# POSTECH-CVLab/PyTorch-StudioGAN

Measured on AMD Instinct MI355X. Metric: images/sec (G+D step) BigGAN ImageNet-128 bs256, higher is better.
Workload: dtype bf16

## Files before the change

include/sgamd.h:

```cpp
#ifndef SGAMD_H
#define SGAMD_H
#include <stdint.h>
#ifdef __cplusplus
extern "C" {
#endif

typedef void* sg_stream_t;

#define SG_DTYPE_F32 0
#define SG_DTYPE_BF16 1
#define SG_DTYPE_F64 2

#define SG_PIX_RELU 1
#define SG_PIX_UPSAMPLE 2
#define SG_PIX_QUAD 4
#define SG_PIX_TRANSPOSED 8
#define SG_EPI_OUT_F32 1
#define SG_EPI_ATOMIC 2
#define SG_EPI_POOL 4
#define SG_EPI_RELU 8
#define SG_EPI_RES_F32 16

const char* sg_last_error(void);
int sg_version(void);
// ... 185 lines not shown
  const float* w;
  const float* u; const float* v; const float* sigma;
  float* dw;
  int rows, cols, Cin, RS, natural, apply_sn, trans;
  int Cin_pad;
} sg_sn_bwd_layer;
int sg_sn_backward(const sg_sn_bwd_layer* layers_dev, const sg_sn_bwd_layer* layers_host, int n, float* work, long long work_floats, sg_stream_t s);

int sg_embedding_fwd(const float* table, const int64_t* idx, float* out, int B, int dim, int num, sg_stream_t s);
int sg_embedding_bwd(const float* dout, const int64_t* idx, float* dtable, int B, int dim, int num, sg_stream_t s);
int sg_relu_sum_hw_fwd(int dtype, const void* x, float* h, int B, int HW, int C, sg_stream_t s);
int sg_relu_sum_hw_bwd(int dtype, const void* x, const float* dh, void* dx, int B, int HW, int C, sg_stream_t s);
int sg_pd_head_fwd(const float* h, const float* w1, const float* b1, const float* emb, float* adv, int B, int C, sg_stream_t s);
int sg_pd_head_bwd(const float* h, const float* w1, const float* emb, const float* dadv, float* dh, float* dw1, float* db1,
                   float* demb, int B, int C, sg_stream_t s);
int sg_loss_d(int kind, const float* real, const float* fake, int B, float* loss, float* d_real, float* d_fake, sg_stream_t s);
int sg_loss_g(int kind, const float* fake, int B, float* loss, float* d_fake, sg_stream_t s);

int sg_interp_rows(const float* real, const float* fake, const float* alpha, float* out, int B, long long n, sg_stream_t s);
int sg_gp_fwd(int kind, const float* grads, int B, long long n, float* norms, float* loss, sg_stream_t s);
int sg_gp_bwd(int kind, const float* grads, const float* norms, const float* gout, float* dgrads, int B, long long n, sg_stream_t s);
int sg_masked_sum_hw(int dtype, const void* t, const void* x, float* out, int B, int HW, int C, sg_stream_t s);

int sg_attn_fused_ok(int B, int HW, int HW4, int Dp, int Cg);
int sg_attn_fwd_fused_ok(int B, int HW, int HW4, int Dp, int Cg);
int sg_attn_fwd_flash_ok(int B, int HW, int HW4, int Dp, int Cg);
int sg_attn_fwd_fused(const void* theta, const void* phi, const void* g, void* P, float* lse, void* O, float* O32, int B, int HW, int HW4, int Dp, int Cg, sg_stream_t s);
int sg_attn_bwd_fused_ok(int B, int HW, int HW4, int Dp, int Cg);
int sg_attn_bwd_fused(const void* theta, const void* phi, const void* g, const void* dO, const float* O32, const float* lse, float* delta, void* dtheta, void* dphi,
                      void* dg, int B, int HW, int HW4, int Dp, int Cg, sg_stream_t s);
int sg_attn_probs_fwd(const void* theta, const void* phi, void* P, float* lse, int B, int HW, int HW4, int Dp, sg_stream_t s);
int sg_attn_ds_bwd(const void* theta, const void* phi, const void* g, const void* dO, const float* lse, void* dS,
                   int B, int HW, int HW4, int Dp, int Cg, sg_stream_t s);

int sg_slice_up_fwd(int dtype, const void* x, void* y, int N, int Hs, int Ws, int ldx, int C, int up, sg_stream_t s);
int sg_slice_up_bwd(int dtype, const void* dy, void* dx, int N, int Hs, int Ws, int ldx, int C, int up, sg_stream_t s);
int sg_copy_channels(int dtype, const void* src, int ld_src, void* dst, int ld_dst, long long rows, int C, sg_stream_t s);

int sg_adam_ema(float* p, const float* g, float* m, float* v, float* ema, long long n, float lr, float beta1, float beta2,
                float eps, float wd, int step, float ema_decay, float grad_scale, sg_stream_t s);
int sg_ema_lerp(const float* src, float* ema, long long n, float decay, sg_stream_t s);

int sg_lecam(const float* real, const float* fake, int B, float ema_real, float ema_fake, float* loss, float* d_real, float* d_fake, sg_stream_t s);
int sg_u8_to_nhwc(int dtype, const uint8_t* x, const uint8_t* flip, void* y, int N, int H, int W, int cpad, sg_stream_t s);

int sg_quantize_resize_normalize(int dtype, const float* x, void* out, uint8_t* quant_out, int N, int C, int H, int W,
                                 int OH, int OW, int quantize, sg_stream_t s);
int sg_pool2d(int dtype, const void* x, void* y, int N, int H, int W, int C, int k, int stride, int pad, int mode, int ldy, int c_off, sg_stream_t s);
int sg_pil_resize_normalize(int dtype, const float* x, void* out, float* tmp, int N, int C, int H, int W, int OH, int OW,
                            const int* bounds_h, const double* kk_h, int ksize_h, const int* bounds_v, const double* kk_v, int ksize_v,
                            int quantize, sg_stream_t s);
int sg_global_avgpool(int dtype, const void* x, float* y, int N, int HW, int C, sg_stream_t s);
int sg_topk_hits(const float* scores, int ld, int ncls, const int64_t* labels, int k, int N, uint8_t* hits, sg_stream_t s);
int sg_topk_select(const float* x, int n, int k, float* vals, int* idx, sg_stream_t s);
int sg_topk_scatter(const float* g, const int* idx, int k, float* dx, int n, sg_stream_t s);
int sg_feat_moments_accumulate(const float* f, int n, int C, double* sum_f, double* sum_ff, sg_stream_t s);
int sg_gather_images_u8(const uint8_t* src, const int64_t* idx, const uint8_t* flip, uint8_t* dst, int B, int H, int W,
                        const int64_t* lab_src, int64_t* lab_dst, sg_stream_t s);
int sg_row_normalize_fwd(const float* x, float* y, float* inv, int rows, int cols, float eps, sg_stream_t s);
int sg_row_normalize_bwd(const float* y, const float* inv, const float* dy, float* dx, int rows, int cols, sg_stream_t s);
int sg_row_dot(const float* a, const float* b, float* p, int rows, int cols, sg_stream_t s);
int sg_row_scale(const float* g, const float* x, float* out, int rows, int cols, int accumulate, sg_stream_t s);
int sg_class_loss(int kind, const float* z, const int64_t* label, int rows, int cols, float* row_loss, float* loss, float* dz, sg_stream_t s);
int sg_contrastive_loss(int kind, const float* S, const float* p, const int64_t* label, int B, float temperature, float m_p,
                        float* row_loss, float* loss, float* dS, float* dp, sg_stream_t s);
int sg_gather_cols(const float* z, const int64_t* label, int rows, int cols, float* out, sg_stream_t s);
// ... 67 lines not shown
```

pytorch-studiogan_amd/_lib.py:

```python
import ctypes as C
import os
import subprocess
import sys

import torch

_HERE = os.path.dirname(os.path.abspath(__file__))
LIB_PATH = os.path.join(_HERE, "libsgamd.so")
if os.environ.get("SG_LIBSGAMD"):
    LIB_PATH = os.path.abspath(os.environ["SG_LIBSGAMD"])
CSRC = os.path.join(_HERE, "csrc")

F32, BF16, F64 = 0, 1, 2
PIX_RELU, PIX_UPSAMPLE, PIX_QUAD, PIX_TRANSPOSED = 1, 2, 4, 8
Q_POOL, Q_UP = 0, 1
EPI_OUT_F32, EPI_ATOMIC, EPI_POOL, EPI_RELU, EPI_RES_F32 = 1, 2, 4, 8, 16

_vp, _i, _f, _ll = C.c_void_p, C.c_int, C.c_float, C.c_longlong


class ConvFwdDesc(C.Structure):
    _fields_ = [("dtype", _i), ("N", _i), ("Hs", _i), ("Ws", _i), ("C", _i), ("ldx", _i), ("Ho", _i), ("Wo", _i), ("Cout", _i),
                ("R", _i), ("S", _i), ("stride", _i), ("pad_h", _i), ("pad_w", _i), ("pix_flags", _i), ("epi_flags", _i),
                ("alpha", _f), ("beta", _f), ("x", _vp), ("w", _vp), ("bias", _vp), ("res", _vp), ("mask", _vp), ("out", _vp),
# ... 116 lines not shown
    "sg_comm_size": [_vp, C.POINTER(_i)],
    "sg_comm_destroy": [_vp],
    "sg_allreduce_flat": [_vp, _vp, _ll, _i, _vp],
    "sg_bn_stats_sync": [_i, _vp, _i, _ll, _i, _vp, _vp, _f, _f, _vp, _vp, _vp, _vp, _vp],
    "sg_set_f32_mode": [_i],
    "sg_get_f32_mode": [],
    "sg_reduce_scatter_flat": [_vp, _vp, _ll, _vp],
    "sg_allgather_flat": [_vp, _vp, _ll, _vp],
    "sg_p2p_create": [_i, _i, _ll, C.POINTER(_vp), _vp],
    "sg_p2p_connect": [_vp, _vp],
    "sg_p2p_destroy": [_vp],
    "sg_p2p_timeouts": [_vp, C.POINTER(_i)],
    "sg_p2p_allreduce_f64": [_vp, _vp, _i, _vp],
    "sg_bn_finalize_p2p": [_vp, _vp, C.c_double, _i, _f, _f, _vp, _vp, _vp, _vp, _vp],
    "sg_bn_stats_sync_p2p": [_i, _vp, _i, _ll, _i, _vp, _vp, _f, _f, _vp, _vp, _vp, _vp, _vp],
    "sg_bn_from_running": [_vp, _vp, _i, _f, _vp, _vp, _vp],
    "sg_bn_apply": [_i, _vp, _vp, _i, _ll, _i, _vp, _vp, _vp, _vp, _i, _i, _vp],
    "sg_bn_bwd_reduce": [_i, _vp, _vp, _i, _ll, _i, _vp, _vp, _vp, _vp, _i, _i, _vp, _vp],
    "sg_bn_bwd_finalize": [_vp, _i, _i, _vp, _i, _vp, _vp, _vp, _vp],
    "sg_bn_bwd_apply": [_i, _vp, _vp, _vp, _i, _ll, _i, _vp, _vp, _vp, _vp, _i, _i, _vp, C.c_double, _i, _vp],
    "sg_bn_bwd_apply_res": [_i, _vp, _vp, _vp, _i, _ll, _i, _vp, _vp, _vp, _vp, _i, _i, _vp, C.c_double, _i, _vp, _vp],
    "sg_bn_bwd2_reduce": [_i, _vp, _vp, _vp, _i, _ll, _i, _vp, _vp, _vp, _vp, _i, _vp, _vp],
    "sg_bn_bwd2_finalize": [_vp, _i, _i, _vp, _vp],
    "sg_bn_bwd2_dgain": [_vp, _vp, C.c_double, _vp, _i, _i, _vp, _vp],
    "sg_bn_bwd2_apply": [_i, _vp, _vp, _vp, _vp, _vp, _i, _ll, _i, _vp, _vp, _vp, _vp, _i, _vp, C.c_double, _i, _vp],
    "sg_attn_fused_ok": [_i, _i, _i, _i, _i],
    "sg_attn_fwd_fused_ok": [_i, _i, _i, _i, _i],
    "sg_attn_fwd_flash_ok": [_i, _i, _i, _i, _i],
    "sg_attn_fwd_fused": [_vp, _vp, _vp, _vp, _vp, _vp, _vp, _i, _i, _i, _i, _i, _vp],
    "sg_attn_bwd_fused_ok": [_i, _i, _i, _i, _i],
    "sg_attn_bwd_fused": [_vp, _vp, _vp, _vp, _vp, _vp, _vp, _vp, _vp, _vp, _i, _i, _i, _i, _i, _vp],
    "sg_attn_probs_fwd": [_vp, _vp, _vp, _vp, _i, _i, _i, _i, _vp],
    "sg_attn_ds_bwd": [_vp, _vp, _vp, _vp, _vp, _vp, _i, _i, _i, _i, _i, _vp],
    "sg_slice_up_fwd": [_i, _vp, _vp, _i, _i, _i, _i, _i, _i, _vp],
    "sg_slice_up_bwd": [_i, _vp, _vp, _i, _i, _i, _i, _i, _i, _vp],
    "sg_copy_channels": [_i, _vp, _i, _vp, _i, _ll, _i, _vp],
    "sg_interp_rows": [_vp, _vp, _vp, _vp, _i, _ll, _vp],
    "sg_gp_fwd": [_i, _vp, _i, _ll, _vp, _vp, _vp],
    "sg_gp_bwd": [_i, _vp, _vp, _vp, _vp, _i, _ll, _vp],
    "sg_masked_sum_hw": [_i, _vp, _vp, _vp, _i, _i, _i, _vp],
    "sg_sn_forward": [_i, _vp, C.POINTER(SnLayer), _i, _f, _vp, _ll, _vp],
    "sg_sn_backward": [_vp, C.POINTER(SnBwdLayer), _i, _vp, _ll, _vp],
    "sg_embedding_fwd": [_vp, _vp, _vp, _i, _i, _i, _vp],
    "sg_embedding_bwd": [_vp, _vp, _vp, _i, _i, _i, _vp],
    "sg_relu_sum_hw_fwd": [_i, _vp, _vp, _i, _i, _i, _vp],
    "sg_relu_sum_hw_bwd": [_i, _vp, _vp, _vp, _i, _i, _i, _vp],
    "sg_pd_head_fwd": [_vp, _vp, _vp, _vp, _vp, _i, _i, _vp],
    "sg_pd_head_bwd": [_vp, _vp, _vp, _vp, _vp, _vp, _vp, _vp, _i, _i, _vp],
    "sg_loss_d": [_i, _vp, _vp, _i, _vp, _vp, _vp, _vp],
    "sg_loss_g": [_i, _vp, _i, _vp, _vp, _vp],
    "sg_adam_ema": [_vp, _vp, _vp, _vp, _vp, _ll, _f, _f, _f, _f, _f, _i, _f, _f, _vp],
    "sg_ema_lerp": [_vp, _vp, _ll, _f, _vp],
    "sg_quantize_resize_normalize": [_i, _vp, _vp, _vp, _i, _i, _i, _i, _i, _i, _i, _vp],
    "sg_pil_resize_normalize": [_i, _vp, _vp, _vp, _i, _i, _i, _i, _i, _i, _vp, _vp, _i, _vp, _vp, _i, _i, _vp],
    "sg_pool2d": [_i, _vp, _vp, _i, _i, _i, _i, _i, _i, _i, _i, _i, _i, _vp],
    "sg_global_avgpool": [_i, _vp, _vp, _i, _i, _i, _vp],
    "sg_feat_moments_accumulate": [_vp, _i, _i, _vp, _vp, _vp],
    "sg_topk_hits": [_vp, _i, _i, _vp, _i, _i, _vp, _vp],
    "sg_row_normalize_fwd": [_vp, _vp, _vp, _i, _i, _f, _vp],
    "sg_row_normalize_bwd": [_vp, _vp, _vp, _vp, _i, _i, _vp],
    "sg_row_dot": [_vp, _vp, _vp, _i, _i, _vp],
    "sg_row_scale": [_vp, _vp, _vp, _i, _i, _i, _vp],
    "sg_class_loss": [_i, _vp, _vp, _i, _i, _vp, _vp, _vp, _vp],
    "sg_contrastive_loss": [_i, _vp, _vp, _vp, _i, _f, _f, _vp, _vp, _vp, _vp, _vp],
    "sg_gather_cols": [_vp, _vp, _i, _i, _vp, _vp],
    "sg_scatter_cols": [_vp, _vp, _i, _i, _vp, _vp],
# ... 120 lines not shown
```

pytorch-studiogan_amd/functional/attention.py:

```python
from ._base import *
from .layout import ConvertFn
from .conv import ConvCfg, ConvDgradFn

class MaxPool2Fn(torch.autograd.Function):

    @staticmethod
    def forward(ctx, x):
        x = _c(x)
        B, H, W, Cc = x.shape
        y = torch.empty((B, (H // 2) * (W // 2), Cc), dtype=x.dtype, device=x.device)
        idx = torch.empty((B, (H // 2) * (W // 2), Cc), dtype=torch.uint8, device=x.device)
        L.call("sg_maxpool2_fwd", L.dt(x), L.ptr(x), Cc, L.ptr(y), Cc, L.ptr(idx), B, H, W, Cc, L.stream())
        ctx.save_for_backward(idx)
        ctx.dims = (B, H, W, Cc)
        return y

    @staticmethod
    def backward(ctx, dy):
        (idx,) = ctx.saved_tensors
        if torch.is_grad_enabled():
            return MaxPool2BwdFn.apply(dy, idx, ctx.dims)
        return _maxpool2_bwd(dy, idx, ctx.dims)


def _maxpool2_bwd(dy, idx, dims):
    B, H, W, Cc = dims
    dy = _c(dy)
    dx = torch.empty((B, H, W, Cc), dtype=dy.dtype, device=dy.device)
    L.call("sg_maxpool2_bwd", L.dt(dy), L.ptr(dy), Cc, L.ptr(idx), L.ptr(dx), Cc, B, H, W, Cc, L.stream())
    return dx


class MaxPool2BwdFn(torch.autograd.Function):
    @staticmethod
    def forward(ctx, dy, idx, dims):
# ... 177 lines not shown
                ins = [t for t, need in zip((theta, phi, g), ctx.needs_input_grad) if need]
                grads = list(torch.autograd.grad(_attn_reference_graph(theta, phi, g, ctx.dims), ins, do, create_graph=True)) if ins else []
            return tuple(grads.pop(0) if need else None for need in ctx.needs_input_grad)
        HW, HW4 = H * W, (H // 2) * (W // 2)
        do = _c(do)
        dev, T = do.device, do.dtype
        sd = L.dt(T)
        if P is None:
            assert lse is not None
            delta = torch.empty((B, HW), dtype=torch.float32, device=dev)
            dtheta = torch.empty((B, H, W, Dp), dtype=T, device=dev)
            dphi = torch.empty((B, HW4, Dp), dtype=T, device=dev)
            dg = torch.empty((B, HW4, Cg), dtype=T, device=dev)
            L.call("sg_attn_bwd_fused", L.ptr(theta), L.ptr(phi), L.ptr(g), L.ptr(do), L.ptr(o32), L.ptr(lse), L.ptr(delta), L.ptr(dtheta), L.ptr(dphi),
                   L.ptr(dg), B, HW, HW4, Dp, Cg, L.stream())
            return dtheta, dphi, dg
        dg = torch.empty((B, HW4, Cg), dtype=T, device=dev)
        gemm_raw(sd, do, 1, Cg, P, 1, HW4, dg, Cg, Cg, HW4, HW, batch=B, p_bs=HW * Cg, q_bs=HW * HW4, out_bs=HW4 * Cg)
        dS = torch.empty((B, HW, HW4), dtype=T, device=dev)
        if lse is not None:
            L.call("sg_attn_ds_bwd", L.ptr(theta), L.ptr(phi), L.ptr(g), L.ptr(do), L.ptr(lse), L.ptr(dS), B, HW, HW4, Dp, Cg, L.stream())
        else:
            dP = torch.empty((B, HW, HW4), dtype=torch.float32, device=dev)
            gemm_raw(sd, g, 0, Cg, do, 0, Cg, dP, HW4, HW4, HW, Cg, batch=B, p_bs=HW4 * Cg, q_bs=HW * Cg, out_bs=HW * HW4, epi_flags=L.EPI_OUT_F32)
            L.call("sg_softmax_rows_bwd", sd, L.ptr(P), L.ptr(dP), L.ptr(dS), B * HW, HW4, L.stream())
            del dP
        dtheta = torch.empty((B, H, W, Dp), dtype=T, device=dev)
        gemm_raw(sd, phi, 1, Dp, dS, 0, HW4, dtheta, Dp, Dp, HW, HW4, batch=B, p_bs=HW4 * Dp, q_bs=HW * HW4, out_bs=HW * Dp)
        dphi = torch.empty((B, HW4, Dp), dtype=T, device=dev)
        gemm_raw(sd, theta, 1, Dp, dS, 1, HW4, dphi, Dp, Dp, HW4, HW, batch=B, p_bs=HW * Dp, q_bs=HW * HW4, out_bs=HW4 * Dp)
        return dtheta, dphi, dg


class AttnOutFn(torch.autograd.Function):

    @staticmethod
    def forward(ctx, x, o, weight, sigma, rt, slot, link=None):
        bank = rt.bank()
        x, o = _c(x), _c(o)
        ctx.link = link
        y = conv2d_raw(o, bank.w_fwd(slot, rt), rt.Cin, rt.rows, 1, 1, res=x, alpha_ptr=sigma)
        ctx.save_for_backward(o, sigma)
        ctx.rt, ctx.slot = rt, slot
        ctx.sigma_param = sigma
        ctx.weight = weight
        return y

    @staticmethod
    def backward(ctx, dy):
        o, sigma = ctx.saved_tensors
        rt, slot = ctx.rt, ctx.slot
        if torch.is_grad_enabled():
            if _param_grad_wanted(ctx.weight, ctx.sigma_param):
                raise NotImplementedError("create_graph=True is supported for input gradients only (WGAN-GP / R1 path)")
            do = ScalePtrFn.apply(ConvDgradFn.apply(dy, o, ctx.weight, rt, slot, ConvCfg(1, 1)), ctx.sigma_param) if ctx.needs_input_grad[1] else None
            return (dy if ctx.needs_input_grad[0] else None), do, None, None, None, None, None
        bank = rt.bank()
        dy = _c(dy)
        N, H, W, Cc = dy.shape
        do = None
        if ctx.needs_input_grad[3]:
            t = conv2d_raw(o, bank.w_fwd(slot, rt), rt.Cin, rt.rows, 1, 1)
            g = ensure_grad(ctx.sigma_param)
            L.call("sg_dot", L.dt(dy), L.ptr(dy), L.ptr(t), dy.numel(), L.ptr(g), 1.0, None, L.stream())
        if ctx.needs_input_grad[1]:
            do = conv2d_raw(dy, bank.w_dgrad(slot, rt), rt.rows, rt.Cin, 1, 1, alpha_ptr=sigma)
        if ctx.needs_input_grad[2]:
            conv2d_wgrad_raw(o, dy, bank.dwt(slot, rt), rt.Cin, rt.rows, 1, 1, H, W, alpha_ptr=sigma)
        dx = dy
        if ctx.link is not None and ctx.link.pending > 0 and ctx.needs_input_grad[0]:
            ctx.link.dx, dx = dy, None
        return dx, do, None, None, None, None, None


__all__ = ['AttnCoreFn', 'AttnOutFn', 'AttnPooledFn', 'BmmFn', 'MaxPool2BwdFn', 'MaxPool2Fn', 'ScalePtrFn', 'SoftmaxRowsBwdFn', 'SoftmaxRowsFn', '_attn_reference_graph', '_maxpool2_bwd']
```

pytorch-studiogan_amd/ops.py:

```python
import torch
import torch.nn as nn
from torch.nn import init
import torch.nn.functional as F_

from . import functional as F
from .bank import get_bank

COMPUTE_DTYPE = torch.float32


def to_nhwc(x, dtype, cpad=0):
    if x.dim() != 4:
        raise RuntimeError("expected a 4-D NCHW tensor")
    if x.dtype == torch.uint8:
        return F.u8_to_nhwc(x, dtype, max(cpad, 3))
    if cpad > x.shape[1]:
        return F.NchwToNhwcFn.apply(x.float(), dtype, cpad)
    if x.dtype == dtype and x.is_contiguous(memory_format=torch.channels_last) and not (x.shape[1] > 1 and x.is_contiguous() and x.shape[2] * x.shape[3] > 1):
        return x.permute(0, 2, 3, 1)
    if x.dtype == torch.float32 and x.is_contiguous():
        return F.NchwToNhwcFn.apply(x, dtype)
    y = x.permute(0, 2, 3, 1).contiguous()
    if y.dtype != dtype:
        y = F.ConvertFn.apply(y, dtype)
# ... 228 lines not shown
            rt_g, rt_b = self.gain._sg_rt, self.bias._sg_rt
            slot = slot if slot is not None else rt_g.bank().current
            gb = F.CbnAffineFn.apply(y, self.gain.master_weight, self.bias.master_weight, rt_g, rt_b, slot, self._ones2)
            return self.bn.forward_nhwc(x, gb, None, relu, link, packed=True)
        gain = self.gain.forward_rt(y, slot, const_bias=self._ones)
        bias = self.bias.forward_rt(y, slot)
        return self.bn.forward_nhwc(x, gain, bias, relu, link)

    def forward(self, x, y):
        _, bank = _root_and_bank(self.gain)
        if self.gain.__dict__.get("_sg_root") is None:
            raise RuntimeError("ConditionalBatchNorm2d must live inside a studiogan_amd backbone (its two linears share the network's bank)")
        return to_nchw(self.forward_nhwc(to_nhwc(x, bank.dtype), y))


class SelfAttention(nn.Module):

    def __init__(self, in_channels, is_generator, MODULES):
        super().__init__()
        self.in_channels = in_channels
        conv = MODULES.g_conv2d if is_generator else MODULES.d_conv2d
        c8, c2 = in_channels // 8, in_channels // 2
        pad8 = (c8 + 7) // 8 * 8
        self.conv1x1_theta = conv(in_channels=in_channels, out_channels=c8, kernel_size=1, stride=1, padding=0, bias=False)
        self.conv1x1_phi = conv(in_channels=in_channels, out_channels=c8, kernel_size=1, stride=1, padding=0, bias=False)
        self.conv1x1_g = conv(in_channels=in_channels, out_channels=c2, kernel_size=1, stride=1, padding=0, bias=False)
        self.conv1x1_attn = conv(in_channels=c2, out_channels=in_channels, kernel_size=1, stride=1, padding=0, bias=False)
        for m in (self.conv1x1_theta, self.conv1x1_phi):
            m._sg_rows_pad = pad8
        self.sigma = nn.Parameter(torch.zeros(1), requires_grad=True)

    def forward_nhwc(self, x, slot=None):
        link = F.GradLink(chain=True) if (F._GRAD_LINK[0] and torch.is_grad_enabled() and x.requires_grad) else None
        theta = self.conv1x1_theta.forward_nhwc(x, slot, link=link)
        phi = self.conv1x1_phi.forward_nhwc(x, slot, link=link)
        g = self.conv1x1_g.forward_nhwc(x, slot, link=link)
        o = F.AttnCoreFn.apply(theta, phi, g)
        rt = self.conv1x1_attn._sg_rt
        slot = slot if slot is not None else rt.bank().current
        return F.AttnOutFn.apply(x, o, self.conv1x1_attn.master_weight, self.sigma, rt, slot, link)

    def forward(self, x):
        _, bank = _root_and_bank(self.conv1x1_theta)
        return to_nchw(self.forward_nhwc(to_nhwc(x, bank.dtype)))


class LeCamEMA(object):

    def __init__(self, init=7777, decay=0.9, start_iter=0):
        self.G_loss = init
        self.D_loss_real = init
        self.D_loss_fake = init
        self.D_real = init
        self.D_fake = init
        self.decay = decay
        self.start_itr = start_iter

    def update(self, cur, mode, itr):
        decay = 0.0 if itr < self.start_itr else self.decay
        if mode not in ("G_loss", "D_loss_real", "D_loss_fake", "D_real", "D_fake"):
            raise ValueError(mode)
        setattr(self, mode, getattr(self, mode) * decay + cur * (1 - decay))


def conv2d(in_channels, out_channels, kernel_size, stride=1, padding=0, dilation=1, groups=1, bias=True):
    return Conv2d(in_channels, out_channels, kernel_size, stride, padding, dilation, groups, bias, sn=False)


def snconv2d(in_channels, out_channels, kernel_size, stride=1, padding=0, dilation=1, groups=1, bias=True):
    return Conv2d(in_channels, out_channels, kernel_size, stride, padding, dilation, groups, bias, sn=True)


# ... 83 lines not shown
```

Measured before the change: 2031.

## Fuse attention theta/phi/g 1x1 projections with 2x2 max-pool into one kernel

Adds an MFMA kernel that computes the theta, phi and g 1x1 convolutions of self-attention in one pass over x, max-pooling phi and g in the epilogue and saving argmax indices. A matching backward kernel un-pools the gradients with those indices, runs the three data-gradient GEMMs together and adds the residual gradient in one pass. SelfAttention now uses this path by default (SG_ATTN_PROJ) and feeds the pooled outputs to AttnPooledFn. The aim is to cut repeated reads of x, the full-resolution phi/g writes, and the separate pooling and launch overhead. In exchange it only covers two shape families, adds uint8 index buffers, and keeps weight gradients on a separate unpool-then-wgrad path.

```diff
diff --git a/include/sgamd.h b/include/sgamd.h
--- a/include/sgamd.h
+++ b/include/sgamd.h
@@ -241,6 +241,12 @@
 int sg_attn_probs_fwd(const void* theta, const void* phi, void* P, float* lse, int B, int HW, int HW4, int Dp, sg_stream_t s);
 int sg_attn_ds_bwd(const void* theta, const void* phi, const void* g, const void* dO, const float* lse, void* dS,
                    int B, int HW, int HW4, int Dp, int Cg, sg_stream_t s);
+
+int sg_attn_proj_ok(int B, int H, int W, int C, int ldx, int Dp, int Cg);
+int sg_attn_proj_fwd(const void* x, int ldx, const void* w_theta, const void* w_phi, const void* w_g, void* theta, void* phi, void* g,
+                     uint8_t* idx_phi, uint8_t* idx_g, int B, int H, int W, int C, int Dp, int Cg, int relu, sg_stream_t s);
+int sg_attn_proj_bwd_data(const void* dtheta, const void* dphi, const void* dg, const uint8_t* idx_phi, const uint8_t* idx_g, const void* wd_theta,
+                          const void* wd_phi, const void* wd_g, const void* res, void* dx, int B, int H, int W, int C, int Dp, int Cg, sg_stream_t s);
 
 int sg_slice_up_fwd(int dtype, const void* x, void* y, int N, int Hs, int Ws, int ldx, int C, int up, sg_stream_t s);
 int sg_slice_up_bwd(int dtype, const void* dy, void* dx, int N, int Hs, int Ws, int ldx, int C, int up, sg_stream_t s);
diff --git a/pytorch-studiogan_amd/_lib.py b/pytorch-studiogan_amd/_lib.py
--- a/pytorch-studiogan_amd/_lib.py
+++ b/pytorch-studiogan_amd/_lib.py
@@ -172,6 +172,9 @@
     "sg_attn_bwd_fused": [_vp, _vp, _vp, _vp, _vp, _vp, _vp, _vp, _vp, _vp, _i, _i, _i, _i, _i, _vp],
     "sg_attn_probs_fwd": [_vp, _vp, _vp, _vp, _i, _i, _i, _i, _vp],
     "sg_attn_ds_bwd": [_vp, _vp, _vp, _vp, _vp, _vp, _i, _i, _i, _i, _i, _vp],
+    "sg_attn_proj_ok": [_i, _i, _i, _i, _i, _i, _i],
+    "sg_attn_proj_fwd": [_vp, _i, _vp, _vp, _vp, _vp, _vp, _vp, _vp, _vp, _i, _i, _i, _i, _i, _i, _i, _vp],
+    "sg_attn_proj_bwd_data": [_vp, _vp, _vp, _vp, _vp, _vp, _vp, _vp, _vp, _vp, _i, _i, _i, _i, _i, _i, _vp],
     "sg_slice_up_fwd": [_i, _vp, _vp, _i, _i, _i, _i, _i, _i, _vp],
     "sg_slice_up_bwd": [_i, _vp, _vp, _i, _i, _i, _i, _i, _i, _vp],
     "sg_copy_channels": [_i, _vp, _i, _vp, _i, _ll, _i, _vp],
diff --git a/pytorch-studiogan_amd/csrc/attn_proj.hip b/pytorch-studiogan_amd/csrc/attn_proj.hip
--- /dev/null
+++ b/pytorch-studiogan_amd/csrc/attn_proj.hip
@@ -0,0 +1,442 @@
+#include <stdlib.h>
+#include "common.h"
+#include "../../include/sgamd.h"
+
+namespace {
+
+constexpr unsigned OOR = 0x80000000u;
+
+typedef short s16x2_t __attribute__((ext_vector_type(2)));
+
+__device__ __forceinline__ unsigned quad_pixel(int row, int H, int W, int wshift, int hshift) {
+  const int qd = row >> 2, dy = (row >> 1) & 1, dx = row & 1;
+  const int wq = qd & ((W >> 1) - 1);
+  const int t = qd >> (wshift - 1);
+  const int hq = t & ((H >> 1) - 1);
+  const int n = t >> (hshift - 1);
+  return (unsigned)(n * H + 2 * hq + dy) * (unsigned)W + (unsigned)(2 * wq + dx);
+}
+
+struct ApFwdParams {
+  const bf16_t* x; const bf16_t* wt; const bf16_t* wp; const bf16_t* wg;
+  bf16_t* theta; bf16_t* phi; bf16_t* g; uint8_t* iphi; uint8_t* ig;
+  int C, ldx, H, W, wshift, hshift, J, relu, nrb;
+  unsigned xbytes, tbytes, pbytes, gbytes;
+};
+
+template <int DP8, int CG8, int KS, int NW>
+__global__ __launch_bounds__(64 * NW) void k_attn_proj_fwd(ApFwdParams p) {
+  constexpr int I = (2 * DP8 + CG8) * 8;
+  constexpr int NT = (I + 31) / 32;
+  constexpr int WP = KS * 32 + 16;
+  constexpr int SP = NT * 64 + 16;
+  constexpr int PCH = DP8 + CG8;
+  constexpr int NITT = (32 * DP8 + 63) / 64, NITP = (8 * PCH + 63) / 64;
+  extern __shared__ __attribute__((aligned(16))) char smem[];
+  char* const wsm = smem;
+  const int tid = threadIdx.x, lane = tid & 63;
+  const int wave = __builtin_amdgcn_readfirstlane(tid >> 6);
+  char* const stg = smem + NT * 32 * WP + wave * (32 * SP);
+
+  for (int idx = tid; idx < NT * 32 * 2 * KS; idx += 64 * NW) {
+    const int row = idx / (2 * KS), c = idx - row * (2 * KS);
+    u32x4 v = {0u, 0u, 0u, 0u};
+    if (row < I && c * 8 < p.C) {
+      const bf16_t* src = row < DP8 * 8 ? p.wt + (long long)row * p.C : row < DP8 * 16 ? p.wp + (long long)(row - DP8 * 8) * p.C : p.wg + (long long)(row - DP8 * 16) * p.C;
+      v = *(const u32x4*)(src + c * 8);
+    }
+    *(u32x4*)(wsm + row * WP + c * 16) = v;
+  }
+  __syncthreads();
+
+  const auto rsx = __builtin_amdgcn_make_buffer_rsrc((void*)p.x, 0, (int)p.xbytes, 0x00020000);
+  const auto rst = __builtin_amdgcn_make_buffer_rsrc((void*)p.theta, 0, (int)p.tbytes, 0x00020000);
+  const auto rsp = __builtin_amdgcn_make_buffer_rsrc((void*)p.phi, 0, (int)p.pbytes, 0x00020000);
+  const auto rsg = __builtin_amdgcn_make_buffer_rsrc((void*)p.g, 0, (int)p.gbytes, 0x00020000);
+  const int frow = lane & 31, fhi = lane >> 5;
+  const unsigned ldx2 = 2u * (unsigned)p.ldx;
+  const short fl = p.relu ? (short)0 : (short)-32768;
+  const s16x2_t floor2 = {fl, fl};
+  const int JQ = p.J >> 2;
+
+  auto fetch = [&](int rb, u32x4 (&q)[KS]) {
+    const int row = rb * 32 + frow;
+    const unsigned base = row < p.J ? quad_pixel(row, p.H, p.W, p.wshift, p.hshift) * ldx2 + (unsigned)fhi * 16u : OOR;
+#pragma unroll
+    for (int ks = 0; ks < KS; ks++) {
+      const unsigned off = ((2 * ks + fhi) * 8 < p.C) ? base + (unsigned)ks * 32u : OOR;
+      q[ks] = __builtin_bit_cast(u32x4, __builtin_amdgcn_raw_buffer_load_b128(rsx, (int)off, 0, 0));
+    }
+  };
+
+  auto compute_store = [&](int rb, u32x4 (&q)[KS]) {
+#pragma unroll
+    for (int ks = 0; ks < KS; ks++)
+#pragma unroll
+      for (int e = 0; e < 4; e++) {
+        const uint32_t xw = q[ks][e];
+        s16x2_t t = __builtin_bit_cast(s16x2_t, xw);
+        t = __builtin_elementwise_max(t, floor2);
+        q[ks][e] = __builtin_bit_cast(uint32_t, t);
+      }
+    f32x16 acc[NT];
+#pragma unroll
+    for (int a = 0; a < NT; a++)
+#pragma unroll
+      for (int r = 0; r < 16; r++) acc[a][r] = 0.f;
+#pragma unroll
+    for (int ks = 0; ks < KS; ks++) {
+      const bf16x8_t qf = __builtin_bit_cast(bf16x8_t, q[ks]);
+#pragma unroll
+      for (int a = 0; a < NT; a++) {
+        const u32x4 v = *(const u32x4*)(wsm + (a * 32 + frow) * WP + (2 * ks + fhi) * 16);
+        acc[a] = __builtin_amdgcn_mfma_f32_32x32x16_bf16(__builtin_bit_cast(bf16x8_t, v), qf, acc[a], 0, 0, 0);
+      }
+    }
+    asm volatile("s_waitcnt lgkmcnt(0)" ::: "memory");
+#pragma unroll
+    for (int a = 0; a < NT; a++)
+#pragma unroll
+      for (int g4 = 0; g4 < 4; g4++) {
+        const int il = a * 32 + 8 * g4 + 4 * fhi;
+        u32x2 t;
+        t[0] = pack2bf(acc[a][4 * g4 + 0], acc[a][4 * g4 + 1]);
+        t[1] = pack2bf(acc[a][4 * g4 + 2], acc[a][4 * g4 + 3]);
+        *(u32x2*)(stg + frow * SP + il * 2) = t;
+      }
+    asm volatile("s_waitcnt lgkmcnt(0)" ::: "memory");
+#pragma unroll
+    for (int it = 0; it < NITT; it++) {
+      const int idx = lane + 64 * it;
+      const int r = idx / DP8, c = idx - r * DP8;
+      const int row = rb * 32 + r;
+      const bool ok = idx < 32 * DP8 && row < p.J;
+      const unsigned off = ok ? (quad_pixel(row, p.H, p.W, p.wshift, p.hshift) * DP8 + (unsigned)c) * 16u : OOR;
+      const u32x4 v = *(const u32x4*)(stg + (r & 31) * SP + c * 16);
+      __builtin_amdgcn_raw_buffer_store_b128(v, rst, (int)off, 0, 0);
+    }
+#pragma unroll
+    for (int it = 0; it < NITP; it++) {
+      const int idx = lane + 64 * it;
+      const int qw = (idx / PCH) & 7, cv = idx - (idx / PCH) * PCH;
+      const int Q = rb * 8 + qw;
+      const bool ok = idx < 8 * PCH && Q < JQ;
+      const char* src = stg + (4 * qw) * SP + (DP8 + cv) * 16;
+      const u32x4 r0 = *(const u32x4*)src, r1 = *(const u32x4*)(src + SP), r2 = *(const u32x4*)(src + 2 * SP), r3 = *(const u32x4*)(src + 3 * SP);
+      float v0[8], v1[8], v2[8], v3[8], m[8];
+      unpack16<bf16_t>(r0, v0); unpack16<bf16_t>(r1, v1); unpack16<bf16_t>(r2, v2); unpack16<bf16_t>(r3, v3);
+      uint32_t a_lo = 0, a_hi = 0;
+#pragma unroll
+      for (int e = 0; e < 8; e++) {
+        float mm = v0[e]; uint32_t a = 0;
+        if (v1[e] > mm) { mm = v1[e]; a = 1; }
+        if (v2[e] > mm) { mm = v2[e]; a = 2; }
+        if (v3[e] > mm) { mm = v3[e]; a = 3; }
+        m[e] = mm;
+        if (e < 4) a_lo |= a << (8 * e); else a_hi |= a << (8 * (e - 4));
+      }
+      u32x4 o;
+#pragma unroll
+      for (int d = 0; d < 4; d++) o[d] = (__float_as_uint(m[2 * d]) >> 16) | (__float_as_uint(m[2 * d + 1]) & 0xffff0000u);
+      const bool isphi = cv < DP8;
+      const unsigned offp = (ok && isphi) ? ((unsigned)Q * DP8 + (unsigned)cv) * 16u : OOR;
+      const unsigned offg = (ok && !isphi) ? ((unsigned)Q * CG8 + (unsigned)(cv - DP8)) * 16u : OOR;
+      __builtin_amdgcn_raw_buffer_store_b128(o, rsp, (int)offp, 0, 0);
+      __builtin_amdgcn_raw_buffer_store_b128(o, rsg, (int)offg, 0, 0);
+      if (ok) {
+        uint8_t* ip = isphi ? p.iphi + ((long long)Q * DP8 + cv) * 8 : p.ig + ((long long)Q * CG8 + (cv - DP8)) * 8;
+        const u32x2 av = {a_lo, a_hi};
+        *(u32x2*)ip = av;
+      }
+    }
+  };
+
+  const int stride = gridDim.x * NW;
+  int rb = blockIdx.x * NW + wave;
+  u32x4 qa[KS], qb[KS];
+  if (rb >= p.nrb) return;
+  fetch(rb, qa);
+  while (true) {
+    fetch(rb + stride, qb);
+    compute_store(rb, qa);
+    rb += stride;
+    if (rb >= p.nrb) break;
+    fetch(rb + stride, qa);
+    compute_store(rb, qb);
+    rb += stride;
+    if (rb >= p.nrb) break;
+  }
+}
+
+struct ApBwdParams {
+  const bf16_t* dtheta; const bf16_t* dphi; const bf16_t* dg; const uint8_t* iphi; const uint8_t* ig;
+  const bf16_t* wt; const bf16_t* wp; const bf16_t* wg;
+  const bf16_t* res; bf16_t* dx;
+  int C, H, W, wshift, hshift, J, nrb;
+  unsigned tbytes, pbytes, gbytes, obytes;
+};
+
+template <int DP8, int CG8, int TI, int NP, int NW>
+__global__ __launch_bounds__(64 * NW) void k_attn_proj_bwd(ApBwdParams p) {
+  constexpr int DS = (DP8 + 1) / 2, GS = CG8 / 2;
+  constexpr int KS = 2 * DS + GS;
+  constexpr int BI = TI * NP * 32;
+  constexpr int WP = KS * 32 + 16;
+  constexpr int CP = TI * 64 + 16;
+  constexpr int CPR = TI * 4;
+  constexpr int NIT = (32 * CPR + 63) / 64;
+  extern __shared__ __attribute__((aligned(16))) char smem[];
+  char* const wsm = smem;
+  const int tid = threadIdx.x, lane = tid & 63;
+  const int wave = __builtin_amdgcn_readfirstlane(tid >> 6);
+  char* const stg = smem + BI * WP + wave * (32 * CP);
+
+  for (int idx = tid; idx < BI * 2 * KS; idx += 64 * NW) {
+    const int row = idx / (2 * KS), c = idx - row * (2 * KS);
+    u32x4 v = {0u, 0u, 0u, 0u};
+    if (row < p.C) {
+      if (c < 2 * DS) { if (c < DP8) v = *(const u32x4*)(p.wt + (long long)row * (DP8 * 8) + c * 8); }
+      else if (c < 4 * DS) { if (c - 2 * DS < DP8) v = *(const u32x4*)(p.wp + (long long)row * (DP8 * 8) + (c - 2 * DS) * 8); }
+      else v = *(const u32x4*)(p.wg + (long long)row * (CG8 * 8) + (c - 4 * DS) * 8);
+    }
+    *(u32x4*)(wsm + row * WP + c * 16) = v;
+  }
+  __syncthreads();
+
+  const auto rst = __builtin_amdgcn_make_buffer_rsrc((void*)p.dtheta, 0, (int)p.tbytes, 0x00020000);
+  const auto rsp = __builtin_amdgcn_make_buffer_rsrc((void*)p.dphi, 0, (int)p.pbytes, 0x00020000);
+  const auto rsg = __builtin_amdgcn_make_buffer_rsrc((void*)p.dg, 0, (int)p.gbytes, 0x00020000);
+  const auto rso = __builtin_amdgcn_make_buffer_rsrc((void*)p.dx, 0, (int)p.obytes, 0x00020000);
+  const auto rsr = __builtin_amdgcn_make_buffer_rsrc((void*)(p.res ? p.res : p.dx), 0, (int)p.obytes, 0x00020000);
+  const int frow = lane & 31, fhi = lane >> 5;
+  const bool pre_res = p.res != nullptr;
+  const unsigned C2 = 2u * (unsigned)p.C;
+  const int ncr = (p.C + 7) >> 3;
+
+  struct Frag { u32x4 t[DS]; u32x4 ph[DS]; u32x2 pi[DS]; u32x4 g[GS]; u32x2 gi[GS]; };
+
+  auto fetch = [&](int rb, Frag& f) {
+    const int row = rb * 32 + frow;
+    const bool rok = row < p.J;
+    const unsigned pix = quad_pixel(rok ? row : 0, p.H, p.W, p.wshift, p.hshift);
+    const unsigned Q = (unsigned)(rok ? row : 0) >> 2;
+#pragma unroll
+    for (int s = 0; s < DS; s++) {
+      const int lc = 2 * s + fhi;
+      const bool ok = rok && lc < DP8;
+      f.t[s] = __builtin_bit_cast(u32x4, __builtin_amdgcn_raw_buffer_load_b128(rst, (int)(ok ? (pix * DP8 + (unsigned)lc) * 16u : OOR), 0, 0));
+      f.ph[s] = __builtin_bit_cast(u32x4, __builtin_amdgcn_raw_buffer_load_b128(rsp, (int)(ok ? (Q * DP8 + (unsigned)lc) * 16u : OOR), 0, 0));
+      f.pi[s] = *(const u32x2*)(p.iphi + (ok ? ((long long)Q * DP8 + lc) * 8 : 0));
+    }
+#pragma unroll
+    for (int s = 0; s < GS; s++) {
+      const int lc = 2 * s + fhi;
+      f.g[s] = __builtin_bit_cast(u32x4, __builtin_amdgcn_raw_buffer_load_b128(rsg, (int)(rok ? (Q * CG8 + (unsigned)lc) * 16u : OOR), 0, 0));
+      f.gi[s] = *(const u32x2*)(p.ig + (rok ? ((long long)Q * CG8 + lc) * 8 : 0));
+    }
+  };
+
+  auto unpool = [](u32x4 g, u32x2 av, uint32_t pos) {
+    u32x4 o;
+#pragma unroll
+    for (int d = 0; d < 4; d++) {
+      const uint32_t w = d < 2 ? av[0] : av[1];
+      const uint32_t a0 = (w >> (16 * (d & 1))) & 0xffu, a1 = (w >> (16 * (d & 1) + 8)) & 0xffu;
+      o[d] = (a0 == pos ? (g[d] & 0xffffu) : 0u) | (a1 == pos ? (g[d] & 0xffff0000u) : 0u);
+    }
+    return o;
+  };
+
+  auto compute_store = [&](int rb, Frag& f) {
+    const uint32_t pos = (uint32_t)(frow & 3);
+    u32x4 q[KS];
+#pragma unroll
+    for (int s = 0; s < DS; s++) { q[s] = f.t[s]; q[DS + s] = unpool(f.ph[s], f.pi[s], pos); }
+#pragma unroll
+    for (int s = 0; s < GS; s++) q[2 * DS + s] = unpool(f.g[s], f.gi[s], pos);
+#pragma unroll
+    for (int ps = 0; ps < NP; ps++) {
+      f32x16 acc[TI];
+#pragma unroll
+      for (int a = 0; a < TI; a++)
+#pragma unroll
+        for (int r = 0; r < 16; r++) acc[a][r] = 0.f;
+#pragma unroll
+      for (int ks = 0; ks < KS; ks++) {
+        const bf16x8_t qf = __builtin_bit_cast(bf16x8_t, q[ks]);
+#pragma unroll
+        for (int a = 0; a < TI; a++) {
+          const u32x4 v = *(const u32x4*)(wsm + ((ps * TI + a) * 32 + frow) * WP + (2 * ks + fhi) * 16);
+          acc[a] = __builtin_amdgcn_mfma_f32_32x32x16_bf16(__builtin_bit_cast(bf16x8_t, v), qf, acc[a], 0, 0, 0);
+        }
+      }
+      const int ic0 = ps * TI * 32;
+      const int ncp = ncr - ps * CPR;
+      asm volatile("s_waitcnt lgkmcnt(0)" ::: "memory");
+      if (pre_res) {
+        u32x4 pre[NIT];
+#pragma unroll
+        for (int it = 0; it < NIT; it++) {
+          const int idx = lane + 64 * it;
+          const int r = idx / CPR, c = idx - r * CPR;
+          const int row = rb * 32 + r;
+          const bool ok = idx < 32 * CPR && row < p.J && c < ncp;
+          const unsigned off = ok ? quad_pixel(row, p.H, p.W, p.wshift, p.hshift) * C2 + (unsigned)(ic0 + c * 8) * 2u : OOR;
+          pre[it] = __builtin_bit_cast(u32x4, __builtin_amdgcn_raw_buffer_load_b128(rsr, (int)off, 0, 0));
+        }
+#pragma unroll
+        for (int it = 0; it < NIT; it++) {
+          const int idx = lane + 64 * it;
+          const int r = idx / CPR, c = idx - r * CPR;
+          if (idx < 32 * CPR) *(u32x4*)(stg + r * CP + c * 16) = pre[it];
+        }
+        asm volatile("s_waitcnt lgkmcnt(0)" ::: "memory");
+      }
+#pragma unroll
+      for (int a = 0; a < TI; a++)
+#pragma unroll
+        for (int g4 = 0; g4 < 4; g4++) {
+          const int il = a * 32 + 8 * g4 + 4 * fhi;
+          char* loc = stg + frow * CP + il * 2;
+          float v[4] = {acc[a][4 * g4 + 0], acc[a][4 * g4 + 1], acc[a][4 * g4 + 2], acc[a][4 * g4 + 3]};
+          if (pre_res) {
+            const u32x2 r = *(const u32x2*)loc;
+#pragma unroll
+            for (int e = 0; e < 4; e++) v[e] += bf2f((bf16_t)((r[e >> 1] >> (16 * (e & 1))) & 0xffffu));
+          }
+          u32x2 t;
+          t[0] = pack2bf(v[0], v[1]);
+          t[1] = pack2bf(v[2], v[3]);
+          *(u32x2*)loc = t;
+        }
+      asm volatile("s_waitcnt lgkmcnt(0)" ::: "memory");
+#pragma unroll
+      for (int it = 0; it < NIT; it++) {
+        const int idx = lane + 64 * it;
+        const int r = idx / CPR, c = idx - r * CPR;
+        const int row = rb * 32 + r;
+        const bool ok = idx < 32 * CPR && row < p.J && c < ncp;
+        const unsigned off = ok ? quad_pixel(row, p.H, p.W, p.wshift, p.hshift) * C2 + (unsigned)(ic0 + c * 8) * 2u : OOR;
+        const u32x4 v = *(const u32x4*)(stg + (r & 31) * CP + c * 16);
+        __builtin_amdgcn_raw_buffer_store_b128(v, rso, (int)off, 0, 0);
+      }
+    }
+  };
+
+  const int stride = gridDim.x * NW;
+  int rb = blockIdx.x * NW + wave;
+  if (rb >= p.nrb) return;
+  Frag fa, fb;
+  fetch(rb, fa);
+  while (true) {
+    fetch(rb + stride, fb);
+    compute_store(rb, fa);
+    rb += stride;
+    if (rb >= p.nrb) break;
+    fetch(rb + stride, fa);
+    compute_store(rb, fb);
+    rb += stride;
+    if (rb >= p.nrb) break;
+  }
+}
+
+int ilog2_pow2(int v) {
+  if (v <= 0 || (v & (v - 1))) return -1;
+  int s = 0;
+  while ((1 << s) < v) s++;
+  return s;
+}
+bool al16(const void* p) { return (((uintptr_t)p) & 15) == 0; }
+
+int family(int C, int Dp, int Cg) {
+  if (Dp == 16 && Cg == 48 && C <= 96) return 0;
+  if (Dp == 24 && Cg == 96 && C <= 192) return 1;
+  return -1;
+}
+
+template <typename K> int set_lds(K kern, int lds) {
+  return hipFuncSetAttribute((const void*)kern, hipFuncAttributeMaxDynamicSharedMemorySize, lds) == hipSuccess ? 0 : -1;
+}
+
+}
+
+extern "C" int sg_attn_proj_ok(int B, int H, int W, int C, int ldx, int Dp, int Cg) {
+  if (B <= 0 || ilog2_pow2(H) < 1 || ilog2_pow2(W) < 1 || C <= 0 || C % 8 || ldx % 8 || ldx < C) return 0;
+  if (family(C, Dp, Cg) < 0) return 0;
+  const long long J = (long long)B * H * W;
+  if (J >= (1ll << 30) || J * ldx * 2 >= (1ll << 31) || J * C * 2 >= (1ll << 31)) return 0;
+  return 1;
+}
+
+extern "C" int sg_attn_proj_fwd(const void* x, int ldx, const void* w_theta, const void* w_phi, const void* w_g, void* theta, void* phi, void* g,
+                                uint8_t* idx_phi, uint8_t* idx_g, int B, int H, int W, int C, int Dp, int Cg, int relu, sg_stream_t s) {
+  SG_CHECK(x && w_theta && w_phi && w_g && theta && phi && g && idx_phi && idx_g, "sg_attn_proj_fwd: null");
+  SG_CHECK(sg_attn_proj_ok(B, H, W, C, ldx, Dp, Cg) == 1, "sg_attn_proj_fwd: unsupported shape (ask sg_attn_proj_ok)");
+  SG_CHECK(al16(x) && al16(w_theta) && al16(w_phi) && al16(w_g) && al16(theta) && al16(phi) && al16(g) && !(((uintptr_t)idx_phi | (uintptr_t)idx_g) & 7),
+           "sg_attn_proj_fwd: misaligned pointer");
+  hipStream_t st = (hipStream_t)s;
+  ApFwdParams p;
+  p.x = (const bf16_t*)x; p.wt = (const bf16_t*)w_theta; p.wp = (const bf16_t*)w_phi; p.wg = (const bf16_t*)w_g;
+  p.theta = (bf16_t*)theta; p.phi = (bf16_t*)phi; p.g = (bf16_t*)g; p.iphi = idx_phi; p.ig = idx_g;
+  p.C = C; p.ldx = ldx; p.H = H; p.W = W; p.wshift = ilog2_pow2(W); p.hshift = ilog2_pow2(H);
+  const long long J = (long long)B * H * W;
+  p.J = (int)J; p.relu = relu ? 1 : 0; p.nrb = (int)((J + 31) / 32);
+  p.xbytes = (unsigned)(((J - 1) * ldx + C) * 2); p.tbytes = (unsigned)(J * Dp * 2); p.pbytes = (unsigned)(J / 4 * Dp * 2); p.gbytes = (unsigned)(J / 4 * Cg * 2);
+  const double I = 2.0 * Dp + Cg;
+  const int prof = sg_prof_begin(st, 2.0 * I * (double)J * (double)C, 0);
+  sg_prof_tag(prof, SG_ENG_CONV_SK, 2.0 * ((double)J * C + I * C + (double)J * Dp) + 0.25 * (double)J * (Dp + Cg) * 3.0);
+#define AP_FWD(DP8, CG8, KS, NW)                                                                                     \
+  {                                                                                                                  \
+    constexpr int NT = ((2 * DP8 + CG8) * 8 + 31) / 32;                                                              \
+    constexpr int lds = NT * 32 * (KS * 32 + 16) + NW * 32 * (NT * 64 + 16);                                         \
+    static_assert(lds <= 160 * 1024, "LDS");                                                                         \
+    static bool done = false;                                                                                        \
+    if (!done) { SG_CHECK(set_lds(k_attn_proj_fwd<DP8, CG8, KS, NW>, lds) == 0, "sg_attn_proj_fwd: LDS attribute"); done = true; } \
+    int gx = (p.nrb + NW - 1) / NW;                                                                                  \
+    const int cap = 256 * (8 / NW);                                                                                  \
+    if (gx > cap) gx = cap;                                                                                          \
+    hipLaunchKernelGGL((k_attn_proj_fwd<DP8, CG8, KS, NW>), dim3(gx), dim3(64 * NW), lds, st, p);                    \
+  }
+  if (family(C, Dp, Cg) == 0) AP_FWD(2, 6, 6, 4) else AP_FWD(3, 12, 12, 8)
+#undef AP_FWD
+  sg_prof_end(st, prof);
+  SG_LAUNCH_CHECK();
+  return 0;
+}
+
+extern "C" int sg_attn_proj_bwd_data(const void* dtheta, const void* dphi, const void* dg, const uint8_t* idx_phi, const uint8_t* idx_g, const void* wd_theta,
+                                     const void* wd_phi, const void* wd_g, const void* res, void* dx, int B, int H, int W, int C, int Dp, int Cg, sg_stream_t s) {
+  SG_CHECK(dtheta && dphi && dg && idx_phi && idx_g && wd_theta && wd_phi && wd_g && dx, "sg_attn_proj_bwd_data: null");
+  SG_CHECK(sg_attn_proj_ok(B, H, W, C, C, Dp, Cg) == 1, "sg_attn_proj_bwd_data: unsupported shape (ask sg_attn_proj_ok)");
+  SG_CHECK(al16(dtheta) && al16(dphi) && al16(dg) && al16(wd_theta) && al16(wd_phi) && al16(wd_g) && al16(res) && al16(dx) &&
+           !(((uintptr_t)idx_phi | (uintptr_t)idx_g) & 7), "sg_attn_proj_bwd_data: misaligned pointer");
+  hipStream_t st = (hipStream_t)s;
+  ApBwdParams p;
+  p.dtheta = (const bf16_t*)dtheta; p.dphi = (const bf16_t*)dphi; p.dg = (const bf16_t*)dg; p.iphi = idx_phi; p.ig = idx_g;
+  p.wt = (const bf16_t*)wd_theta; p.wp = (const bf16_t*)wd_phi; p.wg = (const bf16_t*)wd_g;
+  p.res = (const bf16_t*)res; p.dx = (bf16_t*)dx;
+  p.C = C; p.H = H; p.W = W; p.wshift = ilog2_pow2(W); p.hshift = ilog2_pow2(H);
+  const long long J = (long long)B * H * W;
+  p.J = (int)J; p.nrb = (int)((J + 31) / 32);
+  p.tbytes = (unsigned)(J * Dp * 2); p.pbytes = (unsigned)(J / 4 * Dp * 2); p.gbytes = (unsigned)(J / 4 * Cg * 2); p.obytes = (unsigned)(J * C * 2);
+  const double I = 2.0 * Dp + Cg;
+  const int prof = sg_prof_begin(st, 2.0 * I * (double)J * (double)C, 0);
+  sg_prof_tag(prof, SG_ENG_CONV_SK, 2.0 * ((double)J * C * (res ? 2.0 : 1.0) + I * C + (double)J * Dp) + 0.25 * (double)J * (Dp + Cg) * 3.0);
+#define AP_BWD(DP8, CG8, TI, NP, NW)                                                                                 \
+  {                                                                                                                  \
+    constexpr int KS = 2 * ((DP8 + 1) / 2) + CG8 / 2;                                                                \
+    constexpr int lds = TI * NP * 32 * (KS * 32 + 16) + NW * 32 * (TI * 64 + 16);                                    \
+    static_assert(lds <= 160 * 1024, "LDS");                                                                         \
+    static bool done = false;                                                                                        \
+    if (!done) { SG_CHECK(set_lds(k_attn_proj_bwd<DP8, CG8, TI, NP, NW>, lds) == 0, "sg_attn_proj_bwd_data: LDS attribute"); done = true; } \
+    int gx = (p.nrb + NW - 1) / NW;                                                                                  \
+    const int cap = 256 * (8 / NW);                                                                                  \
+    if (gx > cap) gx = cap;                                                                                          \
+    hipLaunchKernelGGL((k_attn_proj_bwd<DP8, CG8, TI, NP, NW>), dim3(gx), dim3(64 * NW), lds, st, p);                \
+  }
+  if (family(C, Dp, Cg) == 0) AP_BWD(2, 6, 3, 1, 4) else AP_BWD(3, 12, 3, 2, 8)
+#undef AP_BWD
+  sg_prof_end(st, prof);
+  SG_LAUNCH_CHECK();
+  return 0;
+}
diff --git a/pytorch-studiogan_amd/functional/attention.py b/pytorch-studiogan_amd/functional/attention.py
--- a/pytorch-studiogan_amd/functional/attention.py
+++ b/pytorch-studiogan_amd/functional/attention.py
@@ -1,6 +1,6 @@
 from ._base import *
 from .layout import ConvertFn
-from .conv import ConvCfg, ConvDgradFn
+from .conv import ConvCfg, ConvDgradFn, ConvFn, _conv_wgrad
 
 class MaxPool2Fn(torch.autograd.Function):
 
@@ -244,6 +244,80 @@
         return dtheta, dphi, dg
 
 
+def attn_proj_on():
+    return os.environ.get("SG_ATTN_PROJ", "1") != "0"
+
+
+def attn_proj_ok(x, rts):
+    rt_t, rt_p, rt_g = rts
+    if x.dtype != torch.bfloat16 or x.dim() != 4 or rt_t.rows_pad != rt_p.rows_pad or any(r.RS != 1 or r.trans or r.cin_pad != x.shape[3] for r in rts):
+        return False
+    B, H, W, Cc = x.shape
+    return L.lib().sg_attn_proj_ok(B, H, W, Cc, Cc, rt_t.rows_pad, rt_g.rows_pad) == 1
+
+
+class AttnProjFn(torch.autograd.Function):
+
+    @staticmethod
+    def forward(ctx, x, w_theta, w_phi, w_g, rts, slot, link=None):
+        x = _c(x)
+        rt_t, rt_p, rt_g = rts
+        bank = rt_t.bank()
+        B, H, W, Cc = x.shape
+        Dp, Cg = rt_t.rows_pad, rt_g.rows_pad
+        ctx.link = link
+        if link is not None and link.chain:
+            link.pending += 1
+        for _ in rts:
+            _tick()
+        HW4 = (H // 2) * (W // 2)
+        theta = torch.empty((B, H, W, Dp), dtype=x.dtype, device=x.device)
+        phi = torch.empty((B, HW4, Dp), dtype=x.dtype, device=x.device)
+        g = torch.empty((B, HW4, Cg), dtype=x.dtype, device=x.device)
+        iphi = torch.empty((B, HW4, Dp), dtype=torch.uint8, device=x.device)
+        ig = torch.empty((B, HW4, Cg), dtype=torch.uint8, device=x.device)
+        L.call("sg_attn_proj_fwd", L.ptr(x), Cc, bank.w_fwd(slot, rt_t), bank.w_fwd(slot, rt_p), bank.w_fwd(slot, rt_g), L.ptr(theta), L.ptr(phi), L.ptr(g),
+               L.ptr(iphi), L.ptr(ig), B, H, W, Cc, Dp, Cg, 0, L.stream())
+        ctx.save_for_backward(x, iphi, ig)
+        ctx.rts, ctx.slot = rts, slot
+        ctx.weights = (w_theta, w_phi, w_g)
+        return theta, phi, g
+
+    @staticmethod
+    def backward(ctx, dtheta, dphi, dg):
+        x, iphi, ig = ctx.saved_tensors
+        rts, slot = ctx.rts, ctx.slot
+        B, H, W, Cc = x.shape
+        cfg = ConvCfg(1, 1)
+        if torch.is_grad_enabled():
+            if not ctx.needs_input_grad[0]:
+                return (None,) * 7
+            with torch.enable_grad():
+                outs = (ConvFn.apply(x, ctx.weights[0], None, None, rts[0], slot, cfg, None),
+                        MaxPool2Fn.apply(ConvFn.apply(x, ctx.weights[1], None, None, rts[1], slot, cfg, None)),
+                        MaxPool2Fn.apply(ConvFn.apply(x, ctx.weights[2], None, None, rts[2], slot, cfg, None)))
+                (dx,) = torch.autograd.grad(outs, [x], [dtheta, dphi, dg], create_graph=True)
+            return (dx,) + (None,) * 6
+        bank = rts[0].bank()
+        Dp, Cg = rts[0].rows_pad, rts[2].rows_pad
+        dtheta, dphi, dg = _c(dtheta), _c(dphi), _c(dg)
+        dx = None
+        skip_dx = ctx.link.take() if ctx.link is not None else None
+        if ctx.needs_input_grad[0]:
+            dx = torch.empty_like(x)
+            L.call("sg_attn_proj_bwd_data", L.ptr(dtheta), L.ptr(dphi), L.ptr(dg), L.ptr(iphi), L.ptr(ig), bank.w_dgrad(slot, rts[0]), bank.w_dgrad(slot, rts[1]),
+                   bank.w_dgrad(slot, rts[2]), L.ptr(skip_dx), L.ptr(dx), B, H, W, Cc, Dp, Cg, L.stream())
+        elif skip_dx is not None:
+            raise RuntimeError("GradLink: a residual gradient was handed over but the attention block's input needs no gradient")
+        if ctx.link is not None and ctx.link.chain:
+            ctx.link.pending -= 1
+        for k, (dy, idx) in enumerate(((dtheta, None), (dphi, iphi), (dg, ig))):
+            if ctx.needs_input_grad[1 + k]:
+                full = dy if idx is None else _maxpool2_bwd(dy, idx, (B, H, W, dy.shape[-1]))
+                _conv_wgrad(x, full, rts[k], slot, cfg)
+        return (dx,) + (None,) * 6
+
+
 class AttnOutFn(torch.autograd.Function):
 
     @staticmethod
@@ -285,4 +359,4 @@
         return dx, do, None, None, None, None, None
 
 
-__all__ = ['AttnCoreFn', 'AttnOutFn', 'AttnPooledFn', 'BmmFn', 'MaxPool2BwdFn', 'MaxPool2Fn', 'ScalePtrFn', 'SoftmaxRowsBwdFn', 'SoftmaxRowsFn', '_attn_reference_graph', '_maxpool2_bwd']
+__all__ = ['AttnCoreFn', 'AttnOutFn', 'AttnPooledFn', 'AttnProjFn', 'attn_proj_ok', 'attn_proj_on', 'BmmFn', 'MaxPool2BwdFn', 'MaxPool2Fn', 'ScalePtrFn', 'SoftmaxRowsBwdFn', 'SoftmaxRowsFn', '_attn_reference_graph', '_maxpool2_bwd']
diff --git a/pytorch-studiogan_amd/ops.py b/pytorch-studiogan_amd/ops.py
--- a/pytorch-studiogan_amd/ops.py
+++ b/pytorch-studiogan_amd/ops.py
@@ -284,12 +284,18 @@
 
     def forward_nhwc(self, x, slot=None):
         link = F.GradLink(chain=True) if (F._GRAD_LINK[0] and torch.is_grad_enabled() and x.requires_grad) else None
-        theta = self.conv1x1_theta.forward_nhwc(x, slot, link=link)
-        phi = self.conv1x1_phi.forward_nhwc(x, slot, link=link)
-        g = self.conv1x1_g.forward_nhwc(x, slot, link=link)
-        o = F.AttnCoreFn.apply(theta, phi, g)
         rt = self.conv1x1_attn._sg_rt
         slot = slot if slot is not None else rt.bank().current
+        convs = (self.conv1x1_theta, self.conv1x1_phi, self.conv1x1_g)
+        rts = tuple(m._sg_rt for m in convs)
+        if F.attn_proj_on() and all(m.bias is None for m in convs) and F.attn_proj_ok(x, rts):
+            theta, phi_p, g_p = F.AttnProjFn.apply(x, convs[0].master_weight, convs[1].master_weight, convs[2].master_weight, rts, slot, link)
+            o = F.AttnPooledFn.apply(theta, phi_p, g_p)
+        else:
+            theta = self.conv1x1_theta.forward_nhwc(x, slot, link=link)
+            phi = self.conv1x1_phi.forward_nhwc(x, slot, link=link)
+            g = self.conv1x1_g.forward_nhwc(x, slot, link=link)
+            o = F.AttnCoreFn.apply(theta, phi, g)
         return F.AttnOutFn.apply(x, o, self.conv1x1_attn.master_weight, self.sigma, rt, slot, link)
 
     def forward(self, x):
```

After: 2074, median of 6. 2.1% higher.
